# bransonf/mosaic

Measured on AMD Instinct MI355X. Metric: PIP-join points/sec (whole node) at H3 res 9, 1/2/4/8 MI355X vs CPU host, higher is better.
Workload: dtype f64

## Files before the change

mosaic_amd/csrc/join_common.h:

```cpp
#pragma once
#include <hip/hip_runtime.h>
#include <stdint.h>

#include "bng_device.h"
#include "pip_device.h"
#include "raster.h"
#include "tiles.h"

using namespace mosaic;

static const int64_t kEmptyKey = INT64_MIN;

struct HashEntry {
    int64_t key;
    uint32_t first;
    uint32_t count;
};

__host__ __device__ inline uint64_t mix64(uint64_t h) {
    h ^= h >> 33;
    h *= 0xff51afd7ed558ccdULL;
    h ^= h >> 33;
    h *= 0xc4ceb9fe1a85ec53ULL;
    h ^= h >> 33;
// ... 93 lines not shown
__device__ inline void emit_hit(const JoinArgs& a, int64_t row, uint32_t key, unsigned int* lds) {
    if (CM == kCountLds)
        atomicAdd(&lds[key], 1u);
    else if (CM == kCountWaveHash)
        wave_hash_add(a, lds, key);
    else
        atomicAdd(&a.counts[key], 1ULL);
    if (PAIRS) {
        unsigned long long idx = atomicAdd(a.pair_count, 1ULL);
        if ((long long)idx < a.pair_cap) {
            a.pair_row[idx] = row;
            a.pair_key[idx] = (int)key;
        }
    }
}

__device__ inline void stage_push(uint32_t* wq, uint32_t& wn, bool mixed, uint32_t rowoff, unsigned long long lt_mask) {
    const unsigned long long mm = __ballot(mixed);
    if (mixed) wq[wn + __popcll(mm & lt_mask)] = rowoff;
    wn += (uint32_t)__popcll(mm);
}
__device__ inline void stage_flush(const JoinArgs& a, uint32_t* wq, uint32_t& wn, int lane, uint32_t min_rows) {
    if (wn < min_rows || wn == 0) return;
    __builtin_amdgcn_fence(__ATOMIC_RELEASE, "wavefront");
    __builtin_amdgcn_wave_barrier();
    __builtin_amdgcn_fence(__ATOMIC_ACQUIRE, "wavefront");
    unsigned long long base = 0;
    if (lane == 0) base = atomicAdd(a.mixq_count, (unsigned long long)wn);
    base = __shfl(base, 0, 64);
    for (uint32_t k = (uint32_t)lane; k < wn; k += 64) a.mixq[base + k] = wq[k];
    __builtin_amdgcn_wave_barrier();
    wn = 0;
}

struct StreamArgs {
    double x0, y0, sxC, syC;
    double gxmax, gymax;
    int32_t cs, qsh, tsh, qs;
    int32_t qnx, tnx;
    int32_t n_quad_words, n_tiles;
    int32_t tb_lds;
    int32_t stage_words;
    const uint32_t* quad;
    const uint32_t* tile_base;
    const uint16_t* csub;
    const uint16_t* blocks;
    uint32_t csub_bytes, blocks_bytes, tile_base_bytes;
    const uint32_t* qrec;
    int32_t n_qrec, n_qrec_words, qrl;
    double sxF, syF, gx0F, gy0F;
    int32_t gxmaxF, gymaxF, fix_ok;
    const uint32_t* tile_lbase;
    const tiles::LineRec* llines;
};
static const int kStageWords = 128;
static const int kCptBufWords = 192;
static const uint32_t kNoLoad = 0x7ffffff0u;

typedef double v2d __attribute__((ext_vector_type(2)));
typedef unsigned int v4u __attribute__((ext_vector_type(4)));

__device__ inline void lds_fill(uint32_t* dst, const uint32_t* __restrict__ src, int n) {
    const int nt = (int)blockDim.x;
    int k = (int)threadIdx.x;
    for (; k + 7 * nt < n; k += 8 * nt) {
        uint32_t v[8];
// ... 19 lines not shown
}

template <int SH0 = 0>
__device__ inline uint32_t quad_lookup(const StreamArgs& s, const uint16_t* quad, const uint32_t* qmask,
                                       const uint16_t* qcode, uint32_t ixC, uint32_t iyC) {
    const uint32_t q = quad[mad_u24(iyC >> (s.qsh + SH0), (uint32_t)s.qnx, ixC >> (s.qsh + SH0))];
    const uint32_t r = q - 0x8000u;
    const bool rec = r < (uint32_t)s.n_qrec;
    const uint32_t sh = (uint32_t)(s.cs + s.qrl + SH0);
    const uint32_t b = (__builtin_amdgcn_ubfe(iyC, sh, 3u) << 3) | __builtin_amdgcn_ubfe(ixC, sh, 3u);
    const uint32_t rr = rec ? r : 0u;
    const uint32_t w = qmask[2u * rr + (b >> 5)];
    const uint32_t c = qcode[rr];
    return (rec && __builtin_amdgcn_ubfe(w, b & 31u, 1u)) ? c : q;
}

static const uint32_t kBngPure = 0x80000000u, kBngLeaf = 0x40000000u;
static const uint32_t kBngLdsGather = 0xFFu;
struct BngStreamArgs {
    int32_t e0, n0, ne, nn, C;
    double inv_div, div, f;
    int32_t idiv;
    float ff;
    const uint32_t* cells;
    const uint16_t* leaf;
    uint32_t cells_bytes, leaf_bytes;
    const uint32_t* lcell;
    int32_t lcell_words, lsh, lnx;
    const uint16_t* lvl;
    uint32_t lvl_bytes;
    int32_t lvl_stride, lvl_cb;
};

const void* stream_kernel_h3(int pipe, bool lds, bool pairs, bool vec);
const void* leaf_kernel(bool lds, bool pairs);
const void* stream_kernel_bng(bool lds, bool pairs, bool vec, bool cpt);
```

mosaic_amd/csrc/join_stream.hip:

```cpp
#include "join_binned.h"
#include "join_common.h"

template <bool LDS_COUNTS, bool PAIRS, bool VEC>
__global__ void __launch_bounds__(1024) __attribute__((amdgpu_waves_per_eu(4))) k_join_stream(JoinArgs a, StreamArgs s) {
    extern __shared__ unsigned int lds[];
    const int nwaves = (int)(blockDim.x >> 6);
    const int ncw = LDS_COUNTS ? a.n_polygons + 64 : 0;
    uint32_t* stage = lds + ncw;
    uint32_t* tb = stage + nwaves * s.stage_words;
    uint32_t* quadw = tb + (s.tb_lds ? s.n_tiles : 0);
    const uint16_t* quad = (const uint16_t*)quadw;
    uint32_t* qmask = quadw + s.n_quad_words;
    const uint16_t* qcode = (const uint16_t*)(qmask + 2 * s.n_qrec);
    lds_fill(quadw, s.quad, s.n_quad_words);
    lds_fill(qmask, s.qrec, s.n_qrec_words);
    if (s.tb_lds)
        lds_fill(tb, s.tile_base, s.n_tiles);
    for (int k = threadIdx.x; k < ncw; k += blockDim.x) lds[k] = 0;
    __syncthreads();
    const __amdgpu_buffer_rsrc_t rsub = stream_rsrc(s.csub, s.csub_bytes);
    const __amdgpu_buffer_rsrc_t rblk = stream_rsrc(s.blocks, s.blocks_bytes);
    const __amdgpu_buffer_rsrc_t rtb = stream_rsrc(s.tile_base, s.tile_base_bytes);
    const int lane = (int)(threadIdx.x & 63);
    const unsigned long long lt_mask = (1ULL << lane) - 1ULL;
    const int wave = __builtin_amdgcn_readfirstlane((int)(threadIdx.x >> 6));
    uint32_t* wq = stage + wave * s.stage_words;
    uint32_t wn = 0;
    const uint32_t cm = (1u << s.cs) - 1u, qm = (1u << s.qs) - 1u, tm = (1u << s.tsh) - 1u;
    const int64_t stride = (int64_t)gridDim.x * blockDim.x * 4;
    int64_t w0 = a.row_lo + ((int64_t)blockIdx.x * blockDim.x + (int64_t)wave * 64) * 4;
    auto row_of = [&](int64_t wb, int k) -> int64_t { return wb + (k >> 1) * 128 + 2 * lane + (k & 1); };
    v2d px[2], py[2];
    auto load4 = [&](int64_t wb) {
        const int64_t r = (wb + 256 <= a.n) ? wb + 2 * lane : a.row_lo;
        px[0] = __builtin_nontemporal_load((const v2d*)(a.x + r));
        px[1] = __builtin_nontemporal_load((const v2d*)(a.x + r + 128));
// ... 57 lines not shown
            const uint32_t loff = (tbv[k] + (n << (2 * s.cs)) + lf) << 1;
            const uint32_t roff = (tbv[k] - 8u * (n + 1u)) << 1;
            leaf[k] = __builtin_amdgcn_raw_buffer_load_b16(rblk, (blk[k] && !line[k]) ? loff : kNoLoad, 0, 0);
            lrec[k] = __builtin_amdgcn_raw_buffer_load_b128(rblk, line[k] ? roff : kNoLoad, 0, 0);
        }
        if (VEC) load4(w0 + stride);
#pragma unroll
        for (int k = 0; k < 4; k++) {
            const float u = (float)(gx[k] - (double)(ixC[k] & ~tm)), v = (float)(gy[k] - (double)(iyC[k] & ~tm));
            const float sv = fmaf(__uint_as_float(lrec[k].x), u, fmaf(__uint_as_float(lrec[k].y), v, __uint_as_float(lrec[k].z)));
            const uint32_t pos = lrec[k].w & 0xffffu, neg = lrec[k].w >> 16;
            uint32_t lc = sv >= 1.0f ? pos : (uint32_t)tiles::kMixed;
            lc = sv <= -1.0f ? neg : lc;
            uint32_t c = line[k] ? lc : (blk[k] ? leaf[k] : code[k]);
            c = fin[k] && c < 0x8000u ? c : (uint32_t)tiles::kMixed;
            code[k] = live[k] ? c : 0u;
        }
#pragma unroll
        for (int k = 0; k < 4; k++) {
            if (LDS_COUNTS && !PAIRS) {
                const uint32_t slot = code[k] - 1u < 0xfffeu ? code[k] - 1u : (uint32_t)(a.n_polygons + lane);
                atomicAdd(&lds[slot], 1u);
            } else if (code[k] - 1u < 0xfffeu) {
                emit_hit<LDS_COUNTS, PAIRS>(a, row_of(w0, k), code[k] - 1u, lds);
            }
        }
        const bool anym = code[0] == tiles::kMixed || code[1] == tiles::kMixed || code[2] == tiles::kMixed ||
                          code[3] == tiles::kMixed;
        if (__ballot(anym)) {
#pragma unroll
            for (int k = 0; k < 4; k++) {
                const bool m = code[k] == tiles::kMixed;
                const unsigned long long mm = __ballot(m);
                if (m) wq[wn + __popcll(mm & lt_mask)] = (uint32_t)(row_of(w0, k) - a.row_lo);
                wn += (uint32_t)__popcll(mm);
                stage_flush(a, wq, wn, lane, 64);
            }
        }
    }
    stage_flush(a, wq, wn, lane, 1);
    if (LDS_COUNTS) {
        __syncthreads();
        for (int k = threadIdx.x; k < a.n_polygons; k += blockDim.x)
            if (lds[k]) atomicAdd(&a.counts[k], (unsigned long long)lds[k]);
    }
}


template <int aux>
__device__ inline uint32_t gather_b16(__amdgpu_buffer_rsrc_t r, bool need, uint32_t off) {
    uint32_t v = 0u;
    if (need) v = __builtin_amdgcn_raw_buffer_load_b16(r, off, 0, aux);
    return v;
}
__device__ inline uint32_t gather_b32(__amdgpu_buffer_rsrc_t r, bool need, uint32_t off) {
    uint32_t v = 0u;
    if (need) v = __builtin_amdgcn_raw_buffer_load_b32(r, off, 0, 0);
    return v;
}
template <int aux>
__device__ inline v4u gather_b128(__amdgpu_buffer_rsrc_t r, bool need, uint32_t off) {
    v4u v = {0u, 0u, 0u, 0u};
    if (need) v = __builtin_amdgcn_raw_buffer_load_b128(r, off, 0, aux);
    return v;
}

struct PipeGroup {
    uint32_t gx[4], gy[4];
    uint32_t tbv[4];
    uint32_t qv[4];
    uint32_t code[4];
    uint32_t leaf[4];
    v4u lrec[4];
};
static const uint32_t kPipeNonFinite = 0x7fffu;
static_assert(tiles::kMaxRasterKeys + 1 < 0x7fff, "key codes stay below kPipeNonFinite");
static const uint32_t kPipeLine = 0x10000u;

template <bool LDS_COUNTS, bool PAIRS>
__global__ void __launch_bounds__(1024) __attribute__((amdgpu_waves_per_eu(4))) k_join_stream_pipe(JoinArgs a, StreamArgs s) {
    extern __shared__ unsigned int lds[];
    const int nwaves = (int)(blockDim.x >> 6);
    const int ncw = LDS_COUNTS ? a.n_polygons + 64 : 0;
    uint32_t* stage = lds + ncw;
    uint32_t* tb = stage + nwaves * s.stage_words;
    uint32_t* quadw = tb + s.n_tiles;
    const uint16_t* quad = (const uint16_t*)quadw;
    uint32_t* qmask = quadw + s.n_quad_words;
    const uint16_t* qcode = (const uint16_t*)(qmask + 2 * s.n_qrec);
    lds_fill(quadw, s.quad, s.n_quad_words);
    lds_fill(qmask, s.qrec, s.n_qrec_words);
    lds_fill(tb, s.tile_base, s.n_tiles);
    for (int k = threadIdx.x; k < ncw; k += blockDim.x) lds[k] = 0;
    __syncthreads();
    const __amdgpu_buffer_rsrc_t rsub = stream_rsrc(s.csub, s.csub_bytes);
    const __amdgpu_buffer_rsrc_t rblk = stream_rsrc(s.blocks, s.blocks_bytes);
    const int lane = (int)(threadIdx.x & 63);
    const unsigned long long lt_mask = (1ULL << lane) - 1ULL;
    const int wave = __builtin_amdgcn_readfirstlane((int)(threadIdx.x >> 6));
    uint32_t* wq = stage + wave * s.stage_words;
    uint32_t wn = 0;
    const uint32_t cm = (1u << s.cs) - 1u, qm = (1u << s.qs) - 1u;
    const double gx0 = -s.x0 * s.sxC, gy0 = -s.y0 * s.syC;
    const uint32_t spill = (uint32_t)(a.n_polygons + lane);
    const int64_t stride = (int64_t)gridDim.x * blockDim.x * 4;
    const int64_t wbase = a.row_lo + ((int64_t)blockIdx.x * blockDim.x + (int64_t)wave * 64) * 4;
    const int64_t T = wbase + 256 <= a.n ? (a.n - 256 - wbase) / stride + 1 : 0;
    auto row_of = [&](int64_t wb, int k) -> int64_t { return wb + (k >> 1) * 128 + 2 * lane + (k & 1); };
    auto stage_a = [&](const double* x, const double* y, const bool* live, bool valid, PipeGroup& g) {
#pragma unroll
        for (int k = 0; k < 4; k++) {
            const bool lv = valid && live[k];
// ... 22 lines not shown
                                __builtin_amdgcn_ubfe(g.gx[k], (uint32_t)tiles::kFixBits, (uint32_t)s.cs);
            const uint32_t loff = (g.tbv[k] + (n << (2 * s.cs)) + lf) << 1;
            const uint32_t roff = (g.tbv[k] - 8u * (n + 1u)) << 1;
            g.leaf[k] = gather_b16<0>(rblk, blk && !line, loff);
            g.lrec[k] = gather_b128<0>(rblk, line, roff);
            g.code[k] = line ? kPipeLine : (blk ? 0u : c);
        }
    };
    auto stage_d = [&](PipeGroup& g, int64_t wb) {
        uint32_t code[4];
#pragma unroll
        for (int k = 0; k < 4; k++) {
            const uint32_t fb = (uint32_t)(s.tsh + tiles::kFixBits);
            const float u = (float)__builtin_amdgcn_ubfe(g.gx[k], 0u, fb) * (1.0f / (float)(1 << tiles::kFixBits));
            const float v = (float)__builtin_amdgcn_ubfe(g.gy[k], 0u, fb) * (1.0f / (float)(1 << tiles::kFixBits));
            const float sv = fmaf(__uint_as_float(g.lrec[k].x), u,
                                  fmaf(__uint_as_float(g.lrec[k].y), v, __uint_as_float(g.lrec[k].z)));
            const uint32_t pos = g.lrec[k].w & 0xffffu, neg = g.lrec[k].w >> 16;
            uint32_t lc = sv >= 1.0f ? pos : (uint32_t)tiles::kMixed;
            lc = sv <= -1.0f ? neg : lc;
            code[k] = g.code[k] == kPipeLine ? lc : (g.code[k] | g.leaf[k]);
        }
#pragma unroll
        for (int k = 0; k < 4; k++) {
            if (LDS_COUNTS && !PAIRS) {
                const uint32_t slot = min(code[k] - 1u, spill);
                atomicAdd(&lds[slot], 1u);
            } else if (code[k] - 1u < kPipeNonFinite - 1u) {
                emit_hit<LDS_COUNTS, PAIRS>(a, row_of(wb, k), code[k] - 1u, lds);
            }
        }
        const uint32_t cmax = max(max(code[0], code[1]), max(code[2], code[3]));
        if (__ballot(cmax >= kPipeNonFinite)) {
#pragma unroll
            for (int k = 0; k < 4; k++) {
                const bool m = code[k] >= kPipeNonFinite;
                const unsigned long long mm = __ballot(m);
                if (m) wq[wn + __popcll(mm & lt_mask)] = (uint32_t)(row_of(wb, k) - a.row_lo);
                wn += (uint32_t)__popcll(mm);
                stage_flush(a, wq, wn, lane, 64);
            }
        }
    };
    struct Coords {
        v2d px[2], py[2];
    };
    auto load4 = [&](Coords& cb, int64_t wb, bool valid) {
        const int64_t r = valid ? wb + 2 * lane : wbase + 2 * lane;
        cb.px[0] = __builtin_nontemporal_load((const v2d*)(a.x + r));
        cb.px[1] = __builtin_nontemporal_load((const v2d*)(a.x + r + 128));
        cb.py[0] = __builtin_nontemporal_load((const v2d*)(a.y + r));
        cb.py[1] = __builtin_nontemporal_load((const v2d*)(a.y + r + 128));
    };
    Coords cb0, cb1;
    PipeGroup g0, g1;
#pragma unroll
    for (int k = 0; k < 4; k++) {
        g0.qv[k] = g1.qv[k] = 0u;
        g0.code[k] = g1.code[k] = 0u;
        g0.tbv[k] = g1.tbv[k] = 0u;
        g0.gx[k] = g1.gx[k] = g0.gy[k] = g1.gy[k] = 0u;
    }
    auto step = [&](auto VALID, int64_t t, PipeGroup& gfin, PipeGroup& gadv, Coords& cb, Coords& cn) {
        const bool all[4] = {true, true, true, true};
        if (t >= 2) stage_d(gfin, wbase + (t - 2) * stride);
        stage_b(gadv);
        const double x[4] = {cb.px[0].x, cb.px[0].y, cb.px[1].x, cb.px[1].y};
        const double y[4] = {cb.py[0].x, cb.py[0].y, cb.py[1].x, cb.py[1].y};
        stage_a(x, y, all, decltype(VALID)::value, gfin);
        load4(cn, wbase + (t + 1) * stride, t + 1 < T);
    };
    if (T > 0) {
        load4(cb0, wbase, true);
        const std::true_type full;
        const std::false_type drain;
        int64_t t = 0;
        for (; t + 2 <= T; t += 2) {
            step(full, t, g0, g1, cb0, cb1);
            step(full, t + 1, g1, g0, cb1, cb0);
        }
        if (t < T) {
            step(full, t, g0, g1, cb0, cb1);
            step(drain, t + 1, g1, g0, cb1, cb0);
            step(drain, t + 2, g0, g1, cb0, cb1);
        } else {
            step(drain, t, g0, g1, cb0, cb1);
            step(drain, t + 1, g1, g0, cb1, cb0);
        }
    }
    const int64_t wt = wbase + T * stride;
    if (wt < a.n) {
        double x[4], y[4];
        bool live[4];
#pragma unroll
        for (int k = 0; k < 4; k++) {
            const int64_t r = row_of(wt, k);
            live[k] = r < a.n;
            x[k] = live[k] ? a.x[r] : 0.0;
            y[k] = live[k] ? a.y[r] : 0.0;
        }
        PipeGroup g;
        stage_a(x, y, live, true, g);
        stage_b(g);
        stage_d(g, wt);
    }
    stage_flush(a, wq, wn, lane, 1);
    if (LDS_COUNTS) {
        __syncthreads();
        for (int k = threadIdx.x; k < a.n_polygons; k += blockDim.x)
            if (lds[k]) atomicAdd(&a.counts[k], (unsigned long long)lds[k]);
    }
}


struct CptSet {
    uint32_t a;
    uint32_t b;
    uint32_t c;
    uint32_t code;
    uint32_t leaf;
    v4u lrec;
};

template <bool LDS_COUNTS, bool PAIRS>
__global__ void __launch_bounds__(1024) __attribute__((amdgpu_waves_per_eu(4))) k_join_stream_cpt(JoinArgs a, StreamArgs s) {
    extern __shared__ unsigned int lds[];
    const int nwaves = (int)(blockDim.x >> 6);
    const int ncw = LDS_COUNTS ? a.n_polygons + 64 : 0;
    uint32_t* stage = lds + ncw;
    uint32_t* cbuf_all = stage + nwaves * s.stage_words;
    uint32_t* tb = cbuf_all + nwaves * kCptBufWords;
    uint32_t* quadw = tb + (s.tb_lds ? s.n_tiles : 0);
    const uint16_t* quad = (const uint16_t*)quadw;
    uint32_t* qmask = quadw + s.n_quad_words;
    const uint16_t* qcode = (const uint16_t*)(qmask + 2 * s.n_qrec);
    lds_fill(quadw, s.quad, s.n_quad_words);
    lds_fill(qmask, s.qrec, s.n_qrec_words);
    if (s.tb_lds) lds_fill(tb, s.tile_base, s.n_tiles);
    for (int k = threadIdx.x; k < ncw; k += blockDim.x) lds[k] = 0;
    __syncthreads();
    const __amdgpu_buffer_rsrc_t rsub = stream_rsrc(s.csub, s.csub_bytes);
    const __amdgpu_buffer_rsrc_t rblk = stream_rsrc(s.blocks, s.blocks_bytes);
    const __amdgpu_buffer_rsrc_t rtb = stream_rsrc(s.tile_base, s.tile_base_bytes);
    const bool tb_lds = s.tb_lds != 0;
    const int lane = (int)(threadIdx.x & 63);
    const unsigned long long lt_mask = (1ULL << lane) - 1ULL;
    const int wave = __builtin_amdgcn_readfirstlane((int)(threadIdx.x >> 6));
    uint32_t* wq = stage + wave * s.stage_words;
    uint32_t* cbuf = cbuf_all + wave * kCptBufWords;
    uint32_t wn = 0;
    constexpr int F = tiles::kFixBits;
    const uint32_t cs = (uint32_t)s.cs, qs = (uint32_t)s.qs;
    const uint32_t lowm = (1u << max(cs + F + qs, (uint32_t)s.tsh + F)) - 1u;
    const uint32_t spill = (uint32_t)(a.n_polygons + lane);
    double gx0v, gy0v;
    __asm__("v_mov_b64 %0, %1" : "=v"(gx0v) : "s"(s.gx0F));
    __asm__("v_mov_b64 %0, %1" : "=v"(gy0v) : "s"(s.gy0F));
    const int64_t stride = (int64_t)gridDim.x * blockDim.x * 4;
    const int64_t wbase = a.row_lo + ((int64_t)blockIdx.x * blockDim.x + (int64_t)wave * 64) * 4;
    const int64_t T = wbase + 256 <= a.n ? (a.n - 256 - wbase) / stride + 1 : 0;
    auto answer = [&](uint32_t code, int64_t row) {
        if (LDS_COUNTS && !PAIRS) {
            atomicAdd(&lds[min(code - 1u, spill)], 1u);
        } else if (code - 1u < kPipeNonFinite - 1u) {
            emit_hit<LDS_COUNTS, PAIRS>(a, row, code - 1u, lds);
        }
    };
    auto set_a = [&](CptSet& z) {
        const uint32_t q = z.c & 0xffffu;
        const uint32_t local = (__builtin_amdgcn_ubfe(z.b, cs + F, qs) << qs) | __builtin_amdgcn_ubfe(z.a, cs + F, qs);
        uint32_t off = (((q & 0x7fffu) << (2 * qs)) + local) << 1;
#ifdef MOSAIC_ABL_GATHER_HIT
        if (MOSAIC_ABL_GATHER_HIT & 4) off &= 0xffeu;
#endif
        z.code = gather_b16<0>(rsub, q >= 0x8000u, off);
        if (!tb_lds) z.leaf = gather_b32(rtb, q >= 0x8000u, (z.c >> 16) << 2);
    };
    auto set_b = [&](CptSet& z) {
        const uint32_t q = z.c & 0xffffu;
        const uint32_t c = q >= 0x8000u ? z.code : q;
        const bool blk = c - 0x8000u < 0x7fffu;
        const bool line = blk && (c & 0x4000u);
        const uint32_t n = c & 0x3fffu;
        const uint32_t lf = (__builtin_amdgcn_ubfe(z.b, (uint32_t)F, cs) << cs) | __builtin_amdgcn_ubfe(z.a, (uint32_t)F, cs);
        const uint32_t tbv = tb_lds ? tb[z.c >> 16] : z.leaf;
        uint32_t loff = (tbv + (n << (2 * cs)) + lf) << 1;
        uint32_t roff = (tbv - 8u * (n + 1u)) << 1;
#ifdef MOSAIC_ABL_GATHER_HIT
#ifdef MOSAIC_ABL_LMASK
        if (MOSAIC_ABL_GATHER_HIT & 1) roff &= (uint32_t)MOSAIC_ABL_LMASK;
#else
        if (MOSAIC_ABL_GATHER_HIT & 1) roff &= 0xff0u;
#endif
        if (MOSAIC_ABL_GATHER_HIT & 2) loff &= 0xffeu;
#endif
        z.leaf = gather_b16<0>(rblk, blk && !line, loff);
        z.lrec = gather_b128<0>(rblk, line, roff);
        z.code = line ? kPipeLine : (blk ? 0u : c);
    };
    auto set_d = [&](CptSet& z, int64_t wb) {
        const uint32_t fb = (uint32_t)s.tsh + (uint32_t)F;
#ifdef MOSAIC_ABL_GATHER_HIT
        __asm__ volatile("" ::"v"(z.lrec.x), "v"(z.lrec.y), "v"(z.lrec.z), "v"(z.lrec.w), "v"(z.leaf));
        if (MOSAIC_ABL_GATHER_HIT & 9) z.lrec = v4u{0u, 0u, __float_as_uint(2.0f), 0x00010001u};
        if (MOSAIC_ABL_GATHER_HIT & 10) z.leaf = z.code == kPipeLine ? z.leaf : 1u;
#endif
        const float u = (float)__builtin_amdgcn_ubfe(z.a, 0u, fb) * (1.0f / (float)(1 << F));
        const float v = (float)__builtin_amdgcn_ubfe(z.b, 0u, fb) * (1.0f / (float)(1 << F));
        const float sv = fmaf(__uint_as_float(z.lrec.x), u, fmaf(__uint_as_float(z.lrec.y), v, __uint_as_float(z.lrec.z)));
        const uint32_t pos = z.lrec.w & 0xffffu, neg = z.lrec.w >> 16;
        uint32_t lc = sv >= 1.0f ? pos : (uint32_t)tiles::kMixed;
        lc = sv <= -1.0f ? neg : lc;
        const uint32_t code = z.code == kPipeLine ? lc : (z.code | z.leaf);
        const uint32_t src = (z.a >> 24) & 63u, k = z.a >> 30;
        const int64_t row = wb + (int64_t)((k >> 1) * 128u + 2u * src + (k & 1u));
        answer(code, row);
        const bool m = code >= kPipeNonFinite;
        if (__ballot(m)) {
            const unsigned long long mm = __ballot(m);
            if (m) wq[wn + __popcll(mm & lt_mask)] = (uint32_t)(row - a.row_lo);
            wn += (uint32_t)__popcll(mm);
            stage_flush(a, wq, wn, lane, 64);
        }
    };
    auto stage_a = [&](const double* x, const double* y, const bool* live, bool valid, CptSet& z, CptSet& z2, bool& two,
                       int64_t wb) {
        uint32_t fa[4], fb[4], fc[4];
        bool pend[4];
#pragma unroll
        for (int k = 0; k < 4; k++) {
            const uint32_t ixC = min(tiles::fix_cvt(fma(x[k], s.sxF, gx0v)), (uint32_t)s.gxmaxF);
            const uint32_t iyC = min(tiles::fix_cvt(fma(y[k], s.syF, gy0v)), (uint32_t)s.gymaxF);
            const uint32_t q0 = quad_lookup<F>(s, quad, qmask, qcode, ixC, iyC);
            const uint32_t q = valid && live[k] ? q0 : 0u;
            const uint32_t tile = mad_u24(iyC >> (s.tsh + F), (uint32_t)s.tnx, ixC >> (s.tsh + F));
            if (LDS_COUNTS && !PAIRS) atomicAdd(&lds[min(q - 1u, spill)], 1u);
            else if (q - 1u < kPipeNonFinite - 1u) emit_hit<LDS_COUNTS, PAIRS>(a, wb + (k >> 1) * 128 + 2 * lane + (k & 1), q - 1u, lds);
            pend[k] = q >= 0x8000u;
            fa[k] = (ixC & lowm) | ((uint32_t)lane << 24) | ((uint32_t)k << 30);
            fb[k] = iyC & lowm;
            fc[k] = q | (tile << 16);
        }
        uint32_t ranks[4], bases[4];
        uint32_t base = 0;
#pragma unroll
        for (int k = 0; k < 4; k++) {
            const unsigned long long m = __ballot(pend[k]);
            ranks[k] = base + __builtin_amdgcn_mbcnt_hi((uint32_t)(m >> 32), __builtin_amdgcn_mbcnt_lo((uint32_t)m, 0u));
            bases[k] = base;
            base += (uint32_t)__popcll(m);
        }
        const uint32_t P = base;
        auto gather_set = [&](uint32_t sv, CptSet& o) {
#pragma unroll
            for (int k = 0; k < 4; k++) {
// ... 66 lines not shown
            step(full, t, z0, y0, two0, z1, y1, two1, cb0, cb1);
            step(full, t + 1, z1, y1, two1, z0, y0, two0, cb1, cb0);
        }
        if (t < T) {
            step(full, t, z0, y0, two0, z1, y1, two1, cb0, cb1);
            step(drain, t + 1, z1, y1, two1, z0, y0, two0, cb1, cb0);
            step(drain, t + 2, z0, y0, two0, z1, y1, two1, cb0, cb1);
        } else {
            step(drain, t, z0, y0, two0, z1, y1, two1, cb0, cb1);
            step(drain, t + 1, z1, y1, two1, z0, y0, two0, cb1, cb0);
        }
    }
    const int64_t wt = wbase + T * stride;
    if (wt < a.n) {
        double x[4], y[4];
        bool live[4];
#pragma unroll
        for (int k = 0; k < 4; k++) {
            const int64_t r = wt + (k >> 1) * 128 + 2 * lane + (k & 1);
            live[k] = r < a.n;
            x[k] = live[k] ? a.x[r] : 0.0;
            y[k] = live[k] ? a.y[r] : 0.0;
        }
        CptSet z, z2;
        bool two = false;
        stage_a(x, y, live, true, z, z2, two, wt);
        set_b(z);
        set_d(z, wt);
        if (two) {
            set_b(z2);
            set_d(z2, wt);
        }
    }
    stage_flush(a, wq, wn, lane, 1);
    if (LDS_COUNTS) {
        __syncthreads();
        for (int k = threadIdx.x; k < a.n_polygons; k += blockDim.x)
            if (lds[k]) atomicAdd(&a.counts[k], (unsigned long long)lds[k]);
    }
}

template <bool LDS_COUNTS, bool PAIRS, bool VEC>
__global__ void __launch_bounds__(1024) __attribute__((amdgpu_waves_per_eu(4))) k_join_stream_bng(JoinArgs a, BngStreamArgs s) {
    extern __shared__ unsigned int lds[];
    const int ncw = LDS_COUNTS ? a.n_polygons + 64 : 0;
    uint32_t* stage = lds + ncw;
    uint32_t* lcw = stage + (int)(blockDim.x >> 6) * kStageWords;
    const uint8_t* lcell = (const uint8_t*)lcw;
    const bool use_lc = s.lcell_words > 0;
    for (int k = threadIdx.x; k < ncw; k += blockDim.x) lds[k] = 0;
    lds_fill(lcw, s.lcell, s.lcell_words);
    __syncthreads();
    const __amdgpu_buffer_rsrc_t rcell = stream_rsrc(s.cells, s.cells_bytes);
    const __amdgpu_buffer_rsrc_t rleaf = stream_rsrc(s.leaf, s.leaf_bytes);
    const int lane = (int)(threadIdx.x & 63);
    const unsigned long long lt_mask = (1ULL << lane) - 1ULL;
    const int wave = __builtin_amdgcn_readfirstlane((int)(threadIdx.x >> 6));
    uint32_t* wq = stage + wave * kStageWords;
    uint32_t wn = 0;
    bool nan_seen = false;
    const int64_t stride = (int64_t)gridDim.x * blockDim.x * 4;
    int64_t w0 = a.row_lo + ((int64_t)blockIdx.x * blockDim.x + (int64_t)wave * 64) * 4;
    auto row_of = [&](int64_t wb, int k) -> int64_t { return wb + (k >> 1) * 128 + 2 * lane + (k & 1); };
    v2d px[2], py[2];
    auto load4 = [&](int64_t wb) {
        const int64_t r = (wb + 256 <= a.n) ? wb + 2 * lane : a.row_lo;
        px[0] = __builtin_nontemporal_load((const v2d*)(a.x + r));
// ... 337 lines not shown
        }
        BngCptSet z;
        uint32_t zb;
        v4u zrec;
        stage_a(x, y, live, true, z, wt);
        set_b(z, zb);
        set_c(z, zb, zrec);
        set_d(z, zrec, wt);
    }
    stage_flush(a, wq, wn, lane, 1);
    if (__ballot(nan_seen) && lane == 0) atomicOr(a.flags, 1u);
    if (LDS_COUNTS) {
        __syncthreads();
        for (int k = threadIdx.x; k < a.n_polygons; k += blockDim.x)
            if (lds[k]) atomicAdd(&a.counts[k], (unsigned long long)lds[k]);
    }
}

template <bool LDS_COUNTS, bool PAIRS>
__global__ void __launch_bounds__(256) k_join_leaf(JoinArgs a, StreamArgs s, uint32_t* q2, unsigned long long* q2_count) {
    extern __shared__ unsigned int lds[];
    if (LDS_COUNTS) {
        for (int k = threadIdx.x; k < a.n_polygons; k += blockDim.x) lds[k] = 0;
        __syncthreads();
    }
    JoinArgs aq = a;
    aq.mixq = q2;
    aq.mixq_count = q2_count;
    uint32_t* wq = lds + (LDS_COUNTS ? a.n_polygons : 0) + (threadIdx.x >> 6) * kStageWords;
    uint32_t wn = 0;
    constexpr int F = tiles::kFixBits;
    const int lane = (int)(threadIdx.x & 63);
    const unsigned long long lt_mask = (1ULL << lane) - 1ULL;
    const uint16_t* quad = (const uint16_t*)s.quad;
    const uint32_t* qmask = s.qrec;
    const uint16_t* qcode = (const uint16_t*)(s.qrec + 2 * s.n_qrec);
    const uint32_t cs = (uint32_t)s.cs, qs = (uint32_t)s.qs, cm = (1u << cs) - 1u, qm = (1u << qs) - 1u;
    const unsigned long long total = *a.mixq_count;
    const unsigned long long stride = (unsigned long long)gridDim.x * blockDim.x;
    for (unsigned long long t0 = (unsigned long long)blockIdx.x * blockDim.x + (threadIdx.x & ~63u); t0 < total; t0 += stride) {
        const unsigned long long t = t0 + (unsigned long long)lane;
        const bool live = t < total;
        const uint32_t off = live ? a.mixq[t] : 0u;
        const int64_t row = a.row_lo + (int64_t)off;
        uint32_t code = tiles::kMixed;
        if (live) {
            const double x = a.x[row], y = a.y[row];
            if (isfinite(x + y)) {
                const uint32_t gix = min(tiles::fix_cvt(fma(x, s.sxF, s.gx0F)), (uint32_t)s.gxmaxF);
                const uint32_t giy = min(tiles::fix_cvt(fma(y, s.syF, s.gy0F)), (uint32_t)s.gymaxF);
                const uint32_t ixC = gix >> F, iyC = giy >> F, ix = ixC >> cs, iy = iyC >> cs;
                const uint32_t q = quad_lookup<F>(s, quad, qmask, qcode, gix, giy);
                const uint32_t e = q < 0x8000u ? q : s.csub[((q & 0x7fffu) << (2 * qs)) + (((iy & qm) << qs) | (ix & qm))];
                code = e;
                if (tiles::sub_is_block(e) && !(e & tiles::kLineBit)) {
                    const uint32_t tile = (iyC >> s.tsh) * (uint32_t)s.tnx + (ixC >> s.tsh);
                    const uint32_t base = s.tile_base[tile];
                    const uint32_t lc = s.blocks[base + ((e & 0x3fffu) << (2 * cs)) + (((iyC & cm) << cs) | (ixC & cm))];
                    code = lc;
                    if (tiles::leaf_is_line(lc)) {
                        const tiles::LineRec lr = s.llines[s.tile_lbase[tile] + (lc & 0x3fffu)];
                        const uint32_t fm = (1u << (cs + F)) - 1u;
                        const float sc = 1.0f / (float)(1 << F);
                        code = tiles::line_code(lr, (float)(gix & fm) * sc, (float)(giy & fm) * sc);
                    }
                } else if (tiles::sub_is_block(e)) {
                    code = tiles::kMixed;
                }
            }
        }
        const bool keep = live && code >= 0x8000u;
        if (live && !keep && code != 0u) {
            if (LDS_COUNTS && !PAIRS) atomicAdd(&lds[code - 1u], 1u);
            else emit_hit<LDS_COUNTS, PAIRS>(a, row, code - 1u, lds);
        }
        stage_push(wq, wn, keep, off, lt_mask);
        stage_flush(aq, wq, wn, lane, 64);
    }
    stage_flush(aq, wq, wn, lane, 1);
    if (LDS_COUNTS) {
        __syncthreads();
        for (int k = threadIdx.x; k < a.n_polygons; k += blockDim.x)
            if (lds[k]) atomicAdd(&a.counts[k], (unsigned long long)lds[k]);
    }
}

const void* leaf_kernel(bool lds, bool pairs) {
    if (pairs) return (const void*)k_join_leaf<false, true>;
    if (lds) return (const void*)k_join_leaf<true, false>;
    return (const void*)k_join_leaf<false, false>;
}

const void* stream_kernel_h3(int pipe, bool lds, bool pairs, bool vec) {
    if (pipe == 2 && vec) {
        if (pairs) return (const void*)k_join_stream_cpt<false, true>;
        if (lds) return (const void*)k_join_stream_cpt<true, false>;
        return (const void*)k_join_stream_cpt<false, false>;
    }
    if (pipe && vec) {
        if (pairs) return (const void*)k_join_stream_pipe<false, true>;
        if (lds) return (const void*)k_join_stream_pipe<true, false>;
        return (const void*)k_join_stream_pipe<false, false>;
    }
    if (pairs) return vec ? (const void*)k_join_stream<false, true, true> : (const void*)k_join_stream<false, true, false>;
    if (lds) return vec ? (const void*)k_join_stream<true, false, true> : (const void*)k_join_stream<true, false, false>;
    return vec ? (const void*)k_join_stream<false, false, true> : (const void*)k_join_stream<false, false, false>;
}

const void* stream_kernel_bng(bool lds, bool pairs, bool vec, bool cpt) {
    if (cpt && vec) {
        if (pairs) return (const void*)k_join_stream_bng_cpt<false, true>;
        if (lds) return (const void*)k_join_stream_bng_cpt<true, false>;
        return (const void*)k_join_stream_bng_cpt<false, false>;
    }
    if (pairs) return vec ? (const void*)k_join_stream_bng<false, true, true> : (const void*)k_join_stream_bng<false, true, false>;
    if (lds) return vec ? (const void*)k_join_stream_bng<true, false, true> : (const void*)k_join_stream_bng<true, false, false>;
    return vec ? (const void*)k_join_stream_bng<false, false, true> : (const void*)k_join_stream_bng<false, false, false>;
}

extern "C" uint64_t mosaic_layout_join_stream(void) { return mosaic_layout_fingerprint(); }
```

mosaic_amd/csrc/mosaic_hip.hip:

```cpp
#include <hip/hip_runtime.h>
#include <hipcub/hipcub.hpp>
#include <stdint.h>
#include <stdio.h>
#include <string.h>

#include <sys/syscall.h>
#include <unistd.h>

#include <algorithm>
#include <atomic>
#include <chrono>
#include <memory>
#include <mutex>
#include <numeric>
#include <string>
#include <sys/mman.h>
#include <dirent.h>
#include <sys/prctl.h>
#include <thread>
#include <unordered_map>
#include <vector>

#include "../../include/mosaic_hip.h"
#include "bng_device.h"
// ... 1764 lines not shown
            if (ev[k]) (void)hipEventDestroy(ev[k]);
            if (p[k]) (void)hipHostFree(p[k]);
            ev[k] = nullptr;
            p[k] = nullptr;
        }
    }
};

struct DevBufGuard {
    std::vector<DevBuf*> bufs;
    ~DevBufGuard() {
        for (DevBuf* b : bufs) b->release();
    }
};

struct Options {
    int jdk = 8;
    int async = 0;
    int block = 256;
    int blocks_per_cu = 8;
    int raster = 16;
    int raster_adaptive = 1;
    int raster_min_segments = 0;
    int lane_edges = 0;
    int tiles = 1;
    int point_raster = 1;
    int raster_sub = 64;
    int raster_cell = 16;
    int raster_quad = 1;
    int raster_lines = 1;
    int raster_tb_lds = 1;
    int raster_leaf_lines = 1;
    int leaf_join = 1;
    int leaf_blocks_per_cu = 2;
    int exact_defer = 0;
    int raster_build = 1;
    int raster_quad_records = 1;
    int stream_block = 1024;
    int bng_cpt = 1;
    int stream_pipe = 2;
    int bng_lds = 1;
    int bng_cell = 32;
    int bng_group_lines = 1;
    int bng_wedges = 1;
    int cell_blocks_per_cu = 256;
    int mixed_blocks_per_cu = 16;
    int mixed_rows = 1;
    int64_t host_chunk = (int64_t)1 << 25;
    int timing = 0;
    int64_t scratch_limit = 0;
    int bin_points = 1;
    int64_t bin_min_rows = (int64_t)1 << 18;
    int64_t bin_chunk = (int64_t)1 << 28;
    int tile_images = 1;
    int64_t exact_cap = 0;
    int bin_spin_cap = 1 << 20;
    int gk_table_log2 = 16;
    int64_t gk_max_cells = (int64_t)1 << 27;
    int dist_tile = 16;
    int64_t dist_small_work = 512;
    int dist_prune = 1;
    int meas_tile = 256;
    int64_t meas_wave_min = 128;
};

struct ThreadCtx : Options {
    int device = 0;
// ... 2326 lines not shown
                per_cu = 1;
            for (int64_t lo = 0; lo < n; lo += chunk) {
                JoinArgs ac = a;
                ac.row_lo = lo;
                ac.n = std::min<int64_t>(n, lo + chunk);
                if (lo > 0) HIP_TRY(hipMemsetAsync(ac.mixq_count, 0, 8, c->stream));
                const void* kfn = kernel_for(aligned && ac.n - lo >= 256);
                const int gs = (int)std::max<int64_t>(1, std::min<int64_t>((ac.n - lo + 4 * blkb - 1) / (4 * blkb),
                                                                           (int64_t)c->n_cu * per_cu));
                void* kargs[] = {&ac, &bs};
                HIP_TRY(hipLaunchKernel(kfn, dim3(gs), dim3(blkb), kargs, shm_b, c->stream));
                if (tstop && lo == 0) HIP_TRY(hipEventRecord(tstop, c->stream));
                const int gm = (int)std::max<int64_t>(1, std::min<int64_t>((ac.n - lo + 4 * c->block - 1) / (4 * c->block),
                                                                           (int64_t)c->n_cu * c->mixed_blocks_per_cu));
#define MOSAIC_MIXED_BNG(R_)                                                                                     \
    do {                                                                                                         \
        if (pairs) hipLaunchKernelGGL((k_join_mixed_bng<false, true, R_>), dim3(gm), dim3(c->block), 0, c->stream, ac); \
        else if (lds) hipLaunchKernelGGL((k_join_mixed_bng<true, false, R_>), dim3(gm), dim3(c->block), shm, c->stream, ac); \
        else hipLaunchKernelGGL((k_join_mixed_bng<false, false, R_>), dim3(gm), dim3(c->block), 0, c->stream, ac); \
    } while (0)
                hipEvent_t mstop = nullptr;
                if (c->timing == 2 && lo == 0 && (rc = timing_begin(c, &mstop))) return rc;
                if (c->mixed_rows == 4) MOSAIC_MIXED_BNG(4);
                else if (c->mixed_rows == 2) MOSAIC_MIXED_BNG(2);
                else MOSAIC_MIXED_BNG(1);
#undef MOSAIC_MIXED_BNG
                if (mstop) HIP_TRY(hipEventRecord(mstop, c->stream));
                HIP_TRY(hipGetLastError());
            }
            tstop = nullptr;
        } else if (stream) {
            const int64_t chunk = ((int64_t)1 << 32) - 256;
            const int64_t rows = std::min<int64_t>(n, chunk);
            if ((rc = c->mix_queue.reserve((size_t)rows * 4 + 16))) return rc;
            a.mixq = (uint32_t*)c->mix_queue.p;
            a.mixq_count = sc + 4;
            const bool leafq = c->leaf_join && sa.llines && sa.fix_ok;
            if (leafq && (rc = c->mix_queue2.reserve((size_t)rows * 4 + 16))) return rc;
            a.exact_inline = c->exact_defer ? 0 : 1;
            exact_inline = !c->exact_defer;
            const bool aligned = (((uintptr_t)dx | (uintptr_t)dy) & 15) == 0;
            auto mode_for = [&](bool vec) -> int {
                int mode = vec && sa.fix_ok ? c->stream_pipe : 0;
                if (mode >= 2 && !(sa.cs + tiles::kFixBits + sa.qs <= 24 && sa.tsh + tiles::kFixBits <= 24 && sa.n_tiles <= 65536 &&
                                   shm_s + (size_t)(blk / 64) * kCptBufWords * 4 <= kStreamLdsMax))
                    mode = 1;
                if (mode == 1 && !sa.tb_lds) mode = 0;
                return mode;
            };
            auto kernel_for = [&](bool vec) -> const void* { return stream_kernel_h3(mode_for(vec), lds, pairs, vec); };
            auto shm_for = [&](bool vec) -> size_t {
                return shm_s + (mode_for(vec) >= 2 ? (size_t)(blk / 64) * kCptBufWords * 4 : 0);
            };
            int per_cu = 0;
            if (hipOccupancyMaxActiveBlocksPerMultiprocessor(&per_cu, kernel_for(true), blk, shm_for(true)) != hipSuccess ||
                per_cu < 1)
                per_cu = 1;
            for (int64_t lo = 0; lo < n; lo += chunk) {
                JoinArgs ac = a;
                ac.row_lo = lo;
                ac.n = std::min<int64_t>(n, lo + chunk);
                const void* kfn = kernel_for(aligned && ac.n - lo >= 256);
                const int mode = mode_for(aligned && ac.n - lo >= 256);
                if (lo == 0) {
                    static const char* const names[3] = {"k_join_stream", "k_join_stream_pipe", "k_join_stream_cpt"};
                    c->last_kernel = names[mode];
                }
                if (lo > 0) HIP_TRY(hipMemsetAsync(ac.mixq_count, 0, 8, c->stream));
                const int gs = (int)std::max<int64_t>(1, std::min<int64_t>((ac.n - lo + 4 * blk - 1) / (4 * blk),
                                                                           (int64_t)c->n_cu * per_cu));
                void* kargs[] = {&ac, &sa};
                HIP_TRY(hipLaunchKernel(kfn, dim3(gs), dim3(blk), kargs, shm_for(aligned && ac.n - lo >= 256), c->stream));
                if (tstop && lo == 0) HIP_TRY(hipEventRecord(tstop, c->stream));
                const int gm = (int)std::max<int64_t>(1, std::min<int64_t>((ac.n - lo + 4 * c->block - 1) / (4 * c->block),
                                                                           (int64_t)c->n_cu * c->mixed_blocks_per_cu));
#define MOSAIC_MIXED(KERNEL, SHM) \
    hipLaunchKernelGGL(KERNEL, dim3(gm), dim3(c->block), SHM, c->stream, ac)
                hipEvent_t mstop = nullptr;
                if (c->timing == 2 && lo == 0 && (rc = timing_begin(c, &mstop))) return rc;
                const int lb = leafq ? std::max(1, c->n_cu * c->leaf_blocks_per_cu) : 0;
                if (leafq) {
                    uint32_t* q2 = (uint32_t*)c->mix_queue2.p;
                    unsigned long long* q2c = sc + 7;
// ... 1523 lines not shown
```

Before: 314.1 billion.

## Carry tile and leaf code in mixed queue to skip leaf-kernel re-lookup

```diff
diff --git a/mosaic_amd/csrc/join_common.h b/mosaic_amd/csrc/join_common.h
--- a/mosaic_amd/csrc/join_common.h
+++ b/mosaic_amd/csrc/join_common.h
@@ -149,6 +149,28 @@
     __builtin_amdgcn_wave_barrier();
     wn = 0;
 }
+__device__ inline void stage_push2(uint32_t* wq, uint32_t& wn, bool mixed, uint32_t rowoff, uint32_t info,
+                                   unsigned long long lt_mask) {
+    const unsigned long long mm = __ballot(mixed);
+    if (mixed) {
+        const uint32_t e = wn + (uint32_t)__popcll(mm & lt_mask);
+        wq[2u * e] = rowoff;
+        wq[2u * e + 1u] = info;
+    }
+    wn += (uint32_t)__popcll(mm);
+}
+__device__ inline void stage_flush2(const JoinArgs& a, uint32_t* wq, uint32_t& wn, int lane, uint32_t min_rows) {
+    if (wn < min_rows || wn == 0) return;
+    __builtin_amdgcn_fence(__ATOMIC_RELEASE, "wavefront");
+    __builtin_amdgcn_wave_barrier();
+    __builtin_amdgcn_fence(__ATOMIC_ACQUIRE, "wavefront");
+    unsigned long long base = 0;
+    if (lane == 0) base = atomicAdd(a.mixq_count, (unsigned long long)wn);
+    base = __shfl(base, 0, 64);
+    for (uint32_t k = (uint32_t)lane; k < 2u * wn; k += 64) a.mixq[2u * base + k] = wq[k];
+    __builtin_amdgcn_wave_barrier();
+    wn = 0;
+}
 
 struct StreamArgs {
     double x0, y0, sxC, syC;
@@ -234,6 +256,6 @@
     int32_t lvl_stride, lvl_cb;
 };
 
-const void* stream_kernel_h3(int pipe, bool lds, bool pairs, bool vec);
+const void* stream_kernel_h3(int pipe, bool lds, bool pairs, bool vec, bool queue2);
 const void* leaf_kernel(bool lds, bool pairs);
 const void* stream_kernel_bng(bool lds, bool pairs, bool vec, bool cpt);
diff --git a/mosaic_amd/csrc/join_stream.hip b/mosaic_amd/csrc/join_stream.hip
--- a/mosaic_amd/csrc/join_stream.hip
+++ b/mosaic_amd/csrc/join_stream.hip
@@ -1,7 +1,7 @@
 #include "join_binned.h"
 #include "join_common.h"
 
-template <bool LDS_COUNTS, bool PAIRS, bool VEC>
+template <bool LDS_COUNTS, bool PAIRS, bool VEC, bool Q2>
 __global__ void __launch_bounds__(1024) __attribute__((amdgpu_waves_per_eu(4))) k_join_stream(JoinArgs a, StreamArgs s) {
     extern __shared__ unsigned int lds[];
     const int nwaves = (int)(blockDim.x >> 6);
@@ -125,13 +125,26 @@
             for (int k = 0; k < 4; k++) {
                 const bool m = code[k] == tiles::kMixed;
                 const unsigned long long mm = __ballot(m);
-                if (m) wq[wn + __popcll(mm & lt_mask)] = (uint32_t)(row_of(w0, k) - a.row_lo);
-                wn += (uint32_t)__popcll(mm);
-                stage_flush(a, wq, wn, lane, 64);
-            }
-        }
-    }
-    stage_flush(a, wq, wn, lane, 1);
+                if (Q2) {
+                    uint32_t lc = tiles::kMixed;
+                    if (m && fin[k] && blk[k] && !line[k]) {
+                        const int64_t r = row_of(w0, k);
+                        const uint32_t gix = min(tiles::fix_cvt(fma(a.x[r], s.sxF, s.gx0F)), (uint32_t)s.gxmaxF);
+                        const uint32_t giy = min(tiles::fix_cvt(fma(a.y[r], s.syF, s.gy0F)), (uint32_t)s.gymaxF);
+                        if ((gix >> tiles::kFixBits) == ixC[k] && (giy >> tiles::kFixBits) == iyC[k]) lc = leaf[k];
+                    }
+                    stage_flush2(a, wq, wn, lane, 65u - (uint32_t)__popcll(mm));
+                    stage_push2(wq, wn, m, (uint32_t)(row_of(w0, k) - a.row_lo), (ta[k] << 16) | lc, lt_mask);
+                } else {
+                    if (m) wq[wn + __popcll(mm & lt_mask)] = (uint32_t)(row_of(w0, k) - a.row_lo);
+                    wn += (uint32_t)__popcll(mm);
+                    stage_flush(a, wq, wn, lane, 64);
+                }
+            }
+        }
+    }
+    if (Q2) stage_flush2(a, wq, wn, lane, 1);
+    else stage_flush(a, wq, wn, lane, 1);
     if (LDS_COUNTS) {
         __syncthreads();
         for (int k = threadIdx.x; k < a.n_polygons; k += blockDim.x)
@@ -170,7 +183,7 @@
 static_assert(tiles::kMaxRasterKeys + 1 < 0x7fff, "key codes stay below kPipeNonFinite");
 static const uint32_t kPipeLine = 0x10000u;
 
-template <bool LDS_COUNTS, bool PAIRS>
+template <bool LDS_COUNTS, bool PAIRS, bool Q2>
 __global__ void __launch_bounds__(1024) __attribute__((amdgpu_waves_per_eu(4))) k_join_stream_pipe(JoinArgs a, StreamArgs s) {
     extern __shared__ unsigned int lds[];
     const int nwaves = (int)(blockDim.x >> 6);
@@ -259,13 +272,26 @@
         }
         const uint32_t cmax = max(max(code[0], code[1]), max(code[2], code[3]));
         if (__ballot(cmax >= kPipeNonFinite)) {
-#pragma unroll
-            for (int k = 0; k < 4; k++) {
-                const bool m = code[k] >= kPipeNonFinite;
-                const unsigned long long mm = __ballot(m);
-                if (m) wq[wn + __popcll(mm & lt_mask)] = (uint32_t)(row_of(wb, k) - a.row_lo);
-                wn += (uint32_t)__popcll(mm);
-                stage_flush(a, wq, wn, lane, 64);
+            if (Q2) {
+                constexpr int SH = tiles::kFixBits;
+#pragma unroll
+                for (int k = 0; k < 4; k++)
+                    code[k] |= (__umul24(g.gy[k] >> (s.tsh + SH), (uint32_t)s.tnx) + (g.gx[k] >> (s.tsh + SH))) << 16;
+#pragma unroll
+                for (int k = 0; k < 4; k++) {
+                    const bool m = (code[k] & 0xffffu) >= kPipeNonFinite;
+                    stage_flush2(a, wq, wn, lane, 65u - (uint32_t)__popcll(__ballot(m)));
+                    stage_push2(wq, wn, m, (uint32_t)(row_of(wb, k) - a.row_lo), code[k], lt_mask);
+                }
+            } else {
+#pragma unroll
+                for (int k = 0; k < 4; k++) {
+                    const bool m = code[k] >= kPipeNonFinite;
+                    const unsigned long long mm = __ballot(m);
+                    if (m) wq[wn + __popcll(mm & lt_mask)] = (uint32_t)(row_of(wb, k) - a.row_lo);
+                    wn += (uint32_t)__popcll(mm);
+                    stage_flush(a, wq, wn, lane, 64);
+                }
             }
         }
     };
@@ -331,7 +357,8 @@
         stage_b(g);
         stage_d(g, wt);
     }
-    stage_flush(a, wq, wn, lane, 1);
+    if (Q2) stage_flush2(a, wq, wn, lane, 1);
+    else stage_flush(a, wq, wn, lane, 1);
     if (LDS_COUNTS) {
         __syncthreads();
         for (int k = threadIdx.x; k < a.n_polygons; k += blockDim.x)
@@ -349,14 +376,14 @@
     v4u lrec;
 };
 
-template <bool LDS_COUNTS, bool PAIRS>
+template <bool LDS_COUNTS, bool PAIRS, bool Q2>
 __global__ void __launch_bounds__(1024) __attribute__((amdgpu_waves_per_eu(4))) k_join_stream_cpt(JoinArgs a, StreamArgs s) {
     extern __shared__ unsigned int lds[];
     const int nwaves = (int)(blockDim.x >> 6);
     const int ncw = LDS_COUNTS ? a.n_polygons + 64 : 0;
     uint32_t* stage = lds + ncw;
-    uint32_t* cbuf_all = stage + nwaves * s.stage_words;
-    uint32_t* tb = cbuf_all + nwaves * kCptBufWords;
+    const int wave_words = s.stage_words + kCptBufWords;
+    uint32_t* tb = stage + nwaves * wave_words;
     uint32_t* quadw = tb + (s.tb_lds ? s.n_tiles : 0);
     const uint16_t* quad = (const uint16_t*)quadw;
     uint32_t* qmask = quadw + s.n_quad_words;
@@ -373,8 +400,8 @@
     const int lane = (int)(threadIdx.x & 63);
     const unsigned long long lt_mask = (1ULL << lane) - 1ULL;
     const int wave = __builtin_amdgcn_readfirstlane((int)(threadIdx.x >> 6));
-    uint32_t* wq = stage + wave * s.stage_words;
-    uint32_t* cbuf = cbuf_all + wave * kCptBufWords;
+    uint32_t* wq = stage + wave * wave_words;
+    uint32_t* cbuf = wq + s.stage_words;
     uint32_t wn = 0;
     constexpr int F = tiles::kFixBits;
     const uint32_t cs = (uint32_t)s.cs, qs = (uint32_t)s.qs;
@@ -421,16 +448,18 @@
 #endif
         if (MOSAIC_ABL_GATHER_HIT & 2) loff &= 0xffeu;
 #endif
-        z.leaf = gather_b16<0>(rblk, blk && !line, loff);
+        uint32_t lf16 = line ? kPipeLine : 0u;
+        if (blk && !line) lf16 = __builtin_amdgcn_raw_buffer_load_b16(rblk, loff, 0, 0);
+        z.leaf = lf16;
         z.lrec = gather_b128<0>(rblk, line, roff);
-        z.code = line ? kPipeLine : (blk ? 0u : c);
+        z.code = (z.c & 0xffff0000u) | (blk ? 0u : c);
     };
     auto set_d = [&](CptSet& z, int64_t wb) {
         const uint32_t fb = (uint32_t)s.tsh + (uint32_t)F;
 #ifdef MOSAIC_ABL_GATHER_HIT
         __asm__ volatile("" ::"v"(z.lrec.x), "v"(z.lrec.y), "v"(z.lrec.z), "v"(z.lrec.w), "v"(z.leaf));
         if (MOSAIC_ABL_GATHER_HIT & 9) z.lrec = v4u{0u, 0u, __float_as_uint(2.0f), 0x00010001u};
-        if (MOSAIC_ABL_GATHER_HIT & 10) z.leaf = z.code == kPipeLine ? z.leaf : 1u;
+        if (MOSAIC_ABL_GATHER_HIT & 10) z.leaf = z.leaf == kPipeLine ? z.leaf : 1u;
 #endif
         const float u = (float)__builtin_amdgcn_ubfe(z.a, 0u, fb) * (1.0f / (float)(1 << F));
         const float v = (float)__builtin_amdgcn_ubfe(z.b, 0u, fb) * (1.0f / (float)(1 << F));
@@ -438,16 +467,22 @@
         const uint32_t pos = z.lrec.w & 0xffffu, neg = z.lrec.w >> 16;
         uint32_t lc = sv >= 1.0f ? pos : (uint32_t)tiles::kMixed;
         lc = sv <= -1.0f ? neg : lc;
-        const uint32_t code = z.code == kPipeLine ? lc : (z.code | z.leaf);
+        const uint32_t code = z.leaf == kPipeLine ? lc : ((z.code & 0xffffu) | z.leaf);
         const uint32_t src = (z.a >> 24) & 63u, k = z.a >> 30;
         const int64_t row = wb + (int64_t)((k >> 1) * 128u + 2u * src + (k & 1u));
         answer(code, row);
         const bool m = code >= kPipeNonFinite;
         if (__ballot(m)) {
             const unsigned long long mm = __ballot(m);
-            if (m) wq[wn + __popcll(mm & lt_mask)] = (uint32_t)(row - a.row_lo);
-            wn += (uint32_t)__popcll(mm);
-            stage_flush(a, wq, wn, lane, 64);
+            if (Q2) {
+                static_assert(kStageWords + kCptBufWords >= 2 * 127, "a full push fits behind a stage that was not flushed");
+                stage_push2(wq, wn, m, (uint32_t)(row - a.row_lo), (z.code & 0xffff0000u) | code, lt_mask);
+                stage_flush2(a, wq, wn, lane, 64);
+            } else {
+                if (m) wq[wn + __popcll(mm & lt_mask)] = (uint32_t)(row - a.row_lo);
+                wn += (uint32_t)__popcll(mm);
+                stage_flush(a, wq, wn, lane, 64);
+            }
         }
     };
     auto stage_a = [&](const double* x, const double* y, const bool* live, bool valid, CptSet& z, CptSet& z2, bool& two,
@@ -580,7 +615,8 @@
             set_d(z2, wt);
         }
     }
-    stage_flush(a, wq, wn, lane, 1);
+    if (Q2) stage_flush2(a, wq, wn, lane, 1);
+    else stage_flush(a, wq, wn, lane, 1);
     if (LDS_COUNTS) {
         __syncthreads();
         for (int k = threadIdx.x; k < a.n_polygons; k += blockDim.x)
@@ -984,42 +1020,26 @@
     constexpr int F = tiles::kFixBits;
     const int lane = (int)(threadIdx.x & 63);
     const unsigned long long lt_mask = (1ULL << lane) - 1ULL;
-    const uint16_t* quad = (const uint16_t*)s.quad;
-    const uint32_t* qmask = s.qrec;
-    const uint16_t* qcode = (const uint16_t*)(s.qrec + 2 * s.n_qrec);
-    const uint32_t cs = (uint32_t)s.cs, qs = (uint32_t)s.qs, cm = (1u << cs) - 1u, qm = (1u << qs) - 1u;
+    const uint2* __restrict__ mixq2 = (const uint2*)a.mixq;
+    const uint32_t fm = (1u << ((uint32_t)s.cs + F)) - 1u;
+    const float sc = 1.0f / (float)(1 << F);
     const unsigned long long total = *a.mixq_count;
     const unsigned long long stride = (unsigned long long)gridDim.x * blockDim.x;
     for (unsigned long long t0 = (unsigned long long)blockIdx.x * blockDim.x + (threadIdx.x & ~63u); t0 < total; t0 += stride) {
         const unsigned long long t = t0 + (unsigned long long)lane;
         const bool live = t < total;
-        const uint32_t off = live ? a.mixq[t] : 0u;
+        uint2 e = {0u, (uint32_t)tiles::kMixed};
+        if (live) e = mixq2[t];
+        const uint32_t off = e.x, lc = e.y & 0xffffu;
         const int64_t row = a.row_lo + (int64_t)off;
         uint32_t code = tiles::kMixed;
-        if (live) {
+        if (live && tiles::leaf_is_line(lc)) {
             const double x = a.x[row], y = a.y[row];
-            if (isfinite(x + y)) {
-                const uint32_t gix = min(tiles::fix_cvt(fma(x, s.sxF, s.gx0F)), (uint32_t)s.gxmaxF);
-                const uint32_t giy = min(tiles::fix_cvt(fma(y, s.syF, s.gy0F)), (uint32_t)s.gymaxF);
-                const uint32_t ixC = gix >> F, iyC = giy >> F, ix = ixC >> cs, iy = iyC >> cs;
-                const uint32_t q = quad_lookup<F>(s, quad, qmask, qcode, gix, giy);
-                const uint32_t e = q < 0x8000u ? q : s.csub[((q & 0x7fffu) << (2 * qs)) + (((iy & qm) << qs) | (ix & qm))];
-                code = e;
-                if (tiles::sub_is_block(e) && !(e & tiles::kLineBit)) {
-                    const uint32_t tile = (iyC >> s.tsh) * (uint32_t)s.tnx + (ixC >> s.tsh);
-                    const uint32_t base = s.tile_base[tile];
-                    const uint32_t lc = s.blocks[base + ((e & 0x3fffu) << (2 * cs)) + (((iyC & cm) << cs) | (ixC & cm))];
-                    code = lc;
-                    if (tiles::leaf_is_line(lc)) {
-                        const tiles::LineRec lr = s.llines[s.tile_lbase[tile] + (lc & 0x3fffu)];
-                        const uint32_t fm = (1u << (cs + F)) - 1u;
-                        const float sc = 1.0f / (float)(1 << F);
-                        code = tiles::line_code(lr, (float)(gix & fm) * sc, (float)(giy & fm) * sc);
-                    }
-                } else if (tiles::sub_is_block(e)) {
-                    code = tiles::kMixed;
-                }
-            }
+            const uint32_t lbase = s.tile_lbase[e.y >> 16];
+            const tiles::LineRec lr = s.llines[lbase + (lc & 0x3fffu)];
+            const uint32_t gix = min(tiles::fix_cvt(fma(x, s.sxF, s.gx0F)), (uint32_t)s.gxmaxF);
+            const uint32_t giy = min(tiles::fix_cvt(fma(y, s.syF, s.gy0F)), (uint32_t)s.gymaxF);
+            code = tiles::line_code(lr, (float)(gix & fm) * sc, (float)(giy & fm) * sc);
         }
         const bool keep = live && code >= 0x8000u;
         if (live && !keep && code != 0u) {
@@ -1043,20 +1063,24 @@
     return (const void*)k_join_leaf<false, false>;
 }
 
-const void* stream_kernel_h3(int pipe, bool lds, bool pairs, bool vec) {
+template <bool Q2>
+static const void* stream_kernel_h3_q(int pipe, bool lds, bool pairs, bool vec) {
     if (pipe == 2 && vec) {
-        if (pairs) return (const void*)k_join_stream_cpt<false, true>;
-        if (lds) return (const void*)k_join_stream_cpt<true, false>;
-        return (const void*)k_join_stream_cpt<false, false>;
+        if (pairs) return (const void*)k_join_stream_cpt<false, true, Q2>;
+        if (lds) return (const void*)k_join_stream_cpt<true, false, Q2>;
+        return (const void*)k_join_stream_cpt<false, false, Q2>;
     }
     if (pipe && vec) {
-        if (pairs) return (const void*)k_join_stream_pipe<false, true>;
-        if (lds) return (const void*)k_join_stream_pipe<true, false>;
-        return (const void*)k_join_stream_pipe<false, false>;
-    }
-    if (pairs) return vec ? (const void*)k_join_stream<false, true, true> : (const void*)k_join_stream<false, true, false>;
-    if (lds) return vec ? (const void*)k_join_stream<true, false, true> : (const void*)k_join_stream<true, false, false>;
-    return vec ? (const void*)k_join_stream<false, false, true> : (const void*)k_join_stream<false, false, false>;
+        if (pairs) return (const void*)k_join_stream_pipe<false, true, Q2>;
+        if (lds) return (const void*)k_join_stream_pipe<true, false, Q2>;
+        return (const void*)k_join_stream_pipe<false, false, Q2>;
+    }
+    if (pairs) return vec ? (const void*)k_join_stream<false, true, true, Q2> : (const void*)k_join_stream<false, true, false, Q2>;
+    if (lds) return vec ? (const void*)k_join_stream<true, false, true, Q2> : (const void*)k_join_stream<true, false, false, Q2>;
+    return vec ? (const void*)k_join_stream<false, false, true, Q2> : (const void*)k_join_stream<false, false, false, Q2>;
+}
+const void* stream_kernel_h3(int pipe, bool lds, bool pairs, bool vec, bool queue2) {
+    return queue2 ? stream_kernel_h3_q<true>(pipe, lds, pairs, vec) : stream_kernel_h3_q<false>(pipe, lds, pairs, vec);
 }
 
 const void* stream_kernel_bng(bool lds, bool pairs, bool vec, bool cpt) {
diff --git a/mosaic_amd/csrc/mosaic_hip.hip b/mosaic_amd/csrc/mosaic_hip.hip
--- a/mosaic_amd/csrc/mosaic_hip.hip
+++ b/mosaic_amd/csrc/mosaic_hip.hip
@@ -1820,7 +1820,7 @@
     int raster_tb_lds = 1;
     int raster_leaf_lines = 1;
     int leaf_join = 1;
-    int leaf_blocks_per_cu = 2;
+    int leaf_blocks_per_cu = 1;
     int exact_defer = 0;
     int raster_build = 1;
     int raster_quad_records = 1;
@@ -4213,10 +4213,10 @@
         } else if (stream) {
             const int64_t chunk = ((int64_t)1 << 32) - 256;
             const int64_t rows = std::min<int64_t>(n, chunk);
-            if ((rc = c->mix_queue.reserve((size_t)rows * 4 + 16))) return rc;
+            const bool leafq = c->leaf_join && sa.llines && sa.fix_ok && sa.n_tiles <= 65536;
+            if ((rc = c->mix_queue.reserve((size_t)rows * (leafq ? 8 : 4) + 16))) return rc;
             a.mixq = (uint32_t*)c->mix_queue.p;
             a.mixq_count = sc + 4;
-            const bool leafq = c->leaf_join && sa.llines && sa.fix_ok;
             if (leafq && (rc = c->mix_queue2.reserve((size_t)rows * 4 + 16))) return rc;
             a.exact_inline = c->exact_defer ? 0 : 1;
             exact_inline = !c->exact_defer;
@@ -4229,7 +4229,7 @@
                 if (mode == 1 && !sa.tb_lds) mode = 0;
                 return mode;
             };
-            auto kernel_for = [&](bool vec) -> const void* { return stream_kernel_h3(mode_for(vec), lds, pairs, vec); };
+            auto kernel_for = [&](bool vec) -> const void* { return stream_kernel_h3(mode_for(vec), lds, pairs, vec, leafq); };
             auto shm_for = [&](bool vec) -> size_t {
                 return shm_s + (mode_for(vec) >= 2 ? (size_t)(blk / 64) * kCptBufWords * 4 : 0);
             };
```

After: 318.7 billion, median of 6. +1.5%, better.
